# nikizadehgfdl/ocean_model_grid_generator

Measured on AMD Instinct MI355X. Metric: supergrid cells/sec (coords+metrics), 1/8° tripolar at 1/2/4/8 MI355X, higher is better.
Workload: dtype f64

## Files before the change

### ocean_model_grid_generator_amd/csrc/ogg_bipolar_dev.h

```cpp
#pragma once
#include <cstdlib>

#include "ogg_common.h"
#include "ogg_math.h"

namespace {

using namespace ogg;

struct BpRow {
    double sphig;
    double beta2_inv;
    double N_inv;
};
struct BpCol {
    double sinla;
    double alpha2;
};

OGG_DEV BpRow bp_row(double phig_in, double rp) {
    BpRow r;
    const double phig = 90 - div_pi180(2 * atan(tan(0.5 * (90 - phig_in) * kPi180) / rp));
    const double pr = phig * kPi180;
    r.sphig = sin(pr);
    const double t = tan(pr);
    r.beta2_inv = t * t;
    const double chig = (90 - phig) * kPi180;
    const double tg = tan(chig / 2);
    const double rden2 = 1.0 / (1 + (rp * tg) * (rp * tg));
    const double N = rp * (1 + tg * tg) * rden2;
    r.N_inv = 1 / N;
    return r;
}

OGG_DEV BpCol bp_col(double lamg, double lon_bp) {
    BpCol c;
    const double tmp = mdist(lamg, lon_bp) * kPi180;
    double s, co;
    sincos(tmp, &s, &co);
    c.sinla = s;
    c.alpha2 = co * co;
    return c;
}

OGG_DEV void bp_point(const BpRow& r, const BpCol& c, double rp, double& phis, double& h_i_inv, double& h_j_inv, double& rden_out) {
    const double rden = 1.0 / (1.0 + c.alpha2 * r.beta2_inv);
    const double A = c.sinla * r.sphig;
    const double chic = acos(A);
    const double t = tan(chic / 2);
    const double rpt = rp * t;
    phis = 90 - div_pi180(2 * atan(rpt));
    const double rden2 = 1.0 / (1 + rpt * rpt);
    const double M_inv = rp * (1 + t * t) * rden2;
    const double cp = cos(phis * kPi180);
    const double cos2phis = cp * cp;
    const double MM = M_inv * M_inv;
    const bool huge = fabs(r.beta2_inv) > kHuge;
    const double rr = rden * rden;
    double hj = cos2phis * c.alpha2 * (1 - c.alpha2) * r.beta2_inv * (1 + r.beta2_inv) * rr + MM * (1 - c.alpha2) * rden;
    if (huge) hj = MM;
    h_j_inv = sqrt(hj) * r.N_inv;
    double hi = cos2phis * (1 + r.beta2_inv) * rr + MM * c.alpha2 * r.beta2_inv * rden;
    if (huge) hi = MM;
    h_i_inv = sqrt(hi);
    rden_out = rden;
}

template <bool GUARD>
OGG_DEV bool bp_point_fast(const BpRow& r, double b1, double bb1, const BpCol& c, double a1, double aa1, double rp2p, double rp2m,
                           double guard_kk, double& q, double& Xn, double& Yn) {
    const double ab = c.alpha2 * r.beta2_inv;
    const double A = c.sinla * r.sphig;
    const double P = 1.0 + ab;
    const double D = fma(rp2m, A, rp2p);
    const double mp = fma(-A, A, 1.0);
    q = P * D;
    Xn = fma(aa1, fma(mp, bb1, r.beta2_inv), a1);
    Yn = fma(ab, P, mp * b1);
    if (!GUARD) return false;
    const double kc = guard_kk * mp;
    const double uid = (mp * b1) * D, ujd = (mp * (aa1 * bb1)) * D;
    return (uid * uid > kc * (Yn * Yn)) || (ujd * ujd > kc * (Xn * Xn));
}

__constant__ double kAsinPoly[12] = {0x1.5555555555380p-3, 0x1.333333336fd5bp-4, 0x1.6db6db41ce4bdp-5, 0x1.f1c72c668963fp-6,
                                     0x1.6e89f0a0adacfp-6, 0x1.1c6c111dccb70p-6, 0x1.c6fa84b77012bp-7, 0x1.8ed60a300c8d2p-7,
                                     0x1.ab3a098a70509p-8, 0x1.4052137024d6ap-6, -0x1.0a5a378a05eafp-6, 0x1.059859fea6a70p-5};

OGG_DEV double asin_unit(double x) {
    const bool hi = x >= 0.5;
    const double h = fma(x, -0.5, 0.5);
    const double r = hi ? h : x * x;
    const double p = r * horner_scalar<12>(kAsinPoly, r);
    double v = fma(x, p, x);
    if (hi) {
        const double y = __builtin_amdgcn_rsq(h);
        const double g0 = h * y, h0 = y * 0.5;
        const double e = fma(-h0, g0, 0.5);
        const double h1 = fma(h0, e, h0), g1 = fma(g0, e, g0);
        const double d = fma(-g1, g1, h);
        const double s0 = fma(d, h1, g1);
        const bool zero = h == 0.0;
        const double s = zero ? h : s0;
        const double ss = s * s;
        const double sse = fma(s, s, -ss);
        const double t0 = h - ss;
        const double t1 = ((h - t0) - ss) - sse;
        const double num = t0 + t1;
        const double den = s * 2.0;
        const double rc0 = __builtin_amdgcn_rcp(den);
        const double rc1 = fma(fma(-den, rc0, 1.0), rc0, rc0);
        const double rc = fma(fma(-den, rc1, 1.0), rc1, rc1);
        const double q0 = num * rc;
        const double q = fma(fma(-den, q0, num), rc, q0);
        const double c = zero ? 0.0 : q;
        const double sh = s + c;
        const double sl = c - (sh - s);
        const double ph = p * sh;
        const double pl = fma(sl, p, fma(sh, p, -ph));
        const double a = ph + pl;
        const double al = pl - (a - ph);
        const double b = sh + a;
        const double bl = a - (b - sh);
        const double w = (sl + al) + bl;
        const double u = b + w;
        const double ul = w - (u - b);
        constexpr double pio4 = 0x1.921fb54442d18p-1, pio4_lo = 0x1.1a62633145c07p-55;
        const double z = pio4 - u;
        const double zl = (((pio4 - z) - u) + pio4_lo) - ul;
        const double res = z + zl;
        v = (x == 1.0) ? 0x1.921fb54442d18p+0 : res + res;
    }
    return v;
}

OGG_DEV double bp_lamc(const BpRow& r, const BpCol& c, double sqrt_rden) {
    double B = c.sinla * sqrt_rden;
    if (fabs(r.beta2_inv) > kHuge) B = 0.0;
    return div_pi180(asin_unit(B));
}

OGG_DEV double bp_lams_select(double lamc, double lamg, double lon_bp) {
    const double dl = lamg - lon_bp;
    if ((dl > 90) && (dl <= 180)) lamc = 180 - lamc;
    if ((dl > 180) && (dl <= 270)) lamc = 180 + lamc;
    if (dl > 270) lamc = 360 - lamc;
    if (dl == 90) lamc = 90;
    if (dl == 270) lamc = 270;
// ... 329 lines not shown
inline unsigned top_row_blocks(const QuadParams& p) {
    if (p.top_out_row < 0) return 0u;
    const long waves = (p.nx + top_cells<N>() - 1) / top_cells<N>();
    return (unsigned)((waves + 3) / 4);
}

template <int N>
OGG_DEV void bipolar_top_row_body(const QuadParams& p, long w) {
    constexpr int M = N - 1, CW = top_cells<N>();
    const int lane = threadIdx.x & 63;
    const long c0 = w * CW;
    if (c0 >= p.nx) return;
    long u = M * c0 + lane;
    if (u > M * p.nx) u = M * p.nx;
    const double iv = lattice_node(p.q, (int)(u % M), u / M);
    const double lon = p.lon_bp + (iv * 360.0) / (double)p.nx;
    const BpCol c = bp_col(lon, p.lon_bp);
    const double jv = lattice_node(p.q, 0, p.ny);
    const double latg = p.lat0_bp + (jv * (90 - p.lat0_bp)) / (double)p.ny;
    const BpRow r = bp_row(latg, p.rp);
    double phis, rden, h_i, h_j;
    bp_point(r, c, p.rp, phis, h_i, h_j, rden);
    const double dx = h_i * 2 * kPi / (double)p.nx;
    double y[N];
#pragma unroll
    for (int k = 0; k < N; ++k) y[k] = __shfl_down(dx, k);
    const int cell = lane / M;
    if (lane % M == 0 && cell < CW && c0 + cell < p.nx) p.dxq[p.top_out_row * p.nx + c0 + cell] = quad_average_1d<N>(y) * p.Re;
}

template <int N>
OGG_DEV void bipolar_tables_body(const QuadParams& p, long bx) {
    constexpr int M = N - 1;
    const long nb_tab = tables_only_blocks<N>(p);
    if (bx >= nb_tab) {
        bipolar_top_row_body<N>(p, (bx - nb_tab) * 4 + (threadIdx.x >> 6));
        return;
    }
    BpRow* row_tab = const_cast<BpRow*>(p.row_tab);
    BpCol* col_tab = const_cast<BpCol*>(p.col_tab);
    const long k = bx * blockDim.x + threadIdx.x;
    const long n_rows = M * p.ny + 2, n_cols = M * p.nx + 1;
    if (k == 0) *p.fix_count = 0u;
    for (long w = k; w < QUAD_LL_CLAIM_WORDS; w += nb_tab * blockDim.x) p.ll_claims[w] = 0u;
    if (k < n_rows) {
        double jv;
        if (k == M * p.ny)
            jv = (double)p.ny - 0.001;
        else if (k == M * p.ny + 1)
            jv = lattice_node(p.q, 0, p.ny);
        else
            jv = lattice_node(p.q, (int)(k % M), k / M);
        const double latg = p.lat0_bp + (jv * (90 - p.lat0_bp)) / (double)p.ny;
        row_tab[k] = bp_row(latg, p.rp);
    } else if (k < n_rows + n_cols) {
        const long u = k - n_rows;
        const double iv = lattice_node(p.q, (int)(u % M), u / M);
        const double lon = p.lon_bp + (iv * 360.0) / (double)p.nx;
        col_tab[u] = bp_col(lon, p.lon_bp);
    }
}

template <int N>
__global__ __launch_bounds__(256) void bipolar_tables_kernel(QuadParams p) {
    bipolar_tables_body<N>(p, blockIdx.x);
}

template <int N>
inline unsigned tables_blocks(const QuadParams& p) {
    return tables_only_blocks<N>(p) + top_row_blocks<N>(p);
}


OGG_DEV void wg_store_aligned(double* __restrict__ dst, int n, const double* buf, int j0, int sgn, int wave, int lane) {
    const int mis = (int)((reinterpret_cast<unsigned long>(dst) >> 3) & 15ul);
    const int j = 64 * wave + lane - mis;
    if (j >= 0 && j < n) dst[j] = buf[j0 + sgn * j];
    const int j2 = 64 * QS_WAVES + lane - mis;
    if (wave == 0 && j2 < n) dst[j2] = buf[j0 + sgn * j2];
}

struct QuadOutLds {
    double v[2][3][QS_WG_CELLS];
};

template <int N, int MODE>
struct RowEval {
    double dx[N];
    double dy0;
    double pr[N];
    int guarded;
};

constexpr int QM_FAST = 0, QM_GUARD = 1, QM_LITERAL = 2;

template <int N, int MODE>
OGG_DEV void eval_lattice_row(const QuadParams& p, const BpRow& r, const BpCol* col, double rp2p, bool want_dx, RowEval<N, MODE>& o) {
    constexpr int M = N - 1;
    constexpr bool FAITHFUL = (MODE == QM_LITERAL);
    if (FAITHFUL) {
#pragma unroll 1
        for (int ii = 0; ii < M; ++ii) {
            BpCol c = col[0];
#pragma unroll
            for (int k = 1; k < M; ++k) {
                c.sinla = (ii == k) ? col[k].sinla : c.sinla;
                c.alpha2 = (ii == k) ? col[k].alpha2 : c.alpha2;
            }
            double phis, rden, h_i, h_j;
            bp_point(r, c, p.rp, phis, h_i, h_j, rden);
            const double dx = h_i * 2 * kPi / (double)p.nx;
            const double dy = h_j * (90 - p.lat0_bp) * kPi180 / (double)p.ny;
#pragma unroll
            for (int k = 0; k < M; ++k) {
                o.dx[k] = (ii == k) ? dx : o.dx[k];
                o.pr[k] = (ii == k) ? dx * dy : o.pr[k];
            }
            if (ii == 0) o.dy0 = dy;
        }
    } else {
        const double b1 = 1 + r.beta2_inv, bb1 = r.beta2_inv * b1, nsy = r.N_inv * p.sy;
        const double cdx = p.cdx, cdy = (2 * p.rp) * nsy, cpr = p.rp2x4 * (p.sx * nsy);
        const double guard_kk = p.guard_kk, rp2m = p.rp2m;
        int g_first = 0, g_any = 0;
#pragma unroll
        for (int ii = 0; ii < M; ++ii) {
            double q, Xn, Yn;
            const double a1 = 1 - col[ii].alpha2;
            const bool g = bp_point_fast<MODE == QM_GUARD>(r, b1, bb1, col[ii], a1, col[ii].alpha2 * a1, rp2p, rp2m, guard_kk, q, Xn, Yn);
            if (ii == 0) g_first = g;
            g_any |= (int)g;
            const double q2 = q * q;
            constexpr double tiny = 1e-290;
            if (ii == 0 || want_dx) {
                const double dx = (Yn * rsqrt_c3(Yn * q2)) * cdx;
                const double dy = (Xn * rsqrt_c3(fmax(Xn * q2, tiny))) * cdy;
                o.dx[ii] = dx;
                o.pr[ii] = dx * dy;
                if (ii == 0) o.dy0 = dy;
            } else {
                const double xy = Xn * Yn;
                o.pr[ii] = (xy * rsqrt_c3(fmax(xy * (q2 * q2), tiny))) * cpr;
            }
        }
        o.guarded = 0;
        if (MODE == QM_GUARD) o.guarded = g_any | wave_next(g_first);
    }
    if (FAITHFUL) o.guarded = 0;
    if (FAITHFUL || want_dx) o.dx[M] = wave_next(o.dx[0]);
    o.pr[M] = wave_next(o.pr[0]);
}

template <int N, int MODE>
OGG_DEV void bipolar_quad_body(const QuadParams& p, const QuadRange& rg, QuadOutLds& out, long wgx, long by) {
    constexpr int M = N - 1;
    constexpr bool FAITHFUL = (MODE == QM_LITERAL);
    const int lane = threadIdx.x & 63, wave = threadIdx.x >> 6;
    const QuadLane ql = quad_lane(rg.cols, wgx, wave, lane);
    if (ql.nv == 0) return;
    const bool active = ql.active;
    const long ci = ql.ci, c0 = ql.c0;
    const int nv = ql.nv;
    const long n_cols_tab = M * p.nx + 1;
    BpCol col[M];
#pragma unroll
    for (int ii = 0; ii < M; ++ii) {
        long u = M * ci + ii;
        if (u > n_cols_tab - 1) u = n_cols_tab - 1;
        col[ii] = p.col_tab[u];
    }
    const bool cell_lane = ql.cell_lane, closing = ql.closing;
    const bool img_col = (MODE == QM_FAST) && ql.img_col;
    const long h2 = p.nx / 2;
    const QuadStores qs = quad_stores(rg.cols, ql, p.nx, MODE == QM_FAST);
    double rp2p = p.rp2p;
    asm volatile("" : "+v"(rp2p));
    RowEval<N, MODE> cur;
    const long r0 = rg.row_begin + by * rg.rows_per_chunk;
    const long r1 = (r0 + rg.rows_per_chunk < rg.row_end) ? r0 + rg.rows_per_chunk : rg.row_end;
    if (active) eval_lattice_row<N, MODE>(p, p.row_tab[(long)M * r0], col, rp2p, true, cur);
    const int slot = wave * QS_CELLS + lane;
    for (long c = r0; c < r1; ++c) {
        double dxq = 0.0, dyq = 0.0, da = 0.0;
        int guarded = 0;
        if (active) {
            dxq = quad_average_1d<N>(cur.dx) * p.Re;
            guarded = cur.guarded;
            double dyc[N];
            double y2[(N <= 3) ? N * N : 1];
            double ysum = 0.0;
#pragma unroll
            for (int k = 0; k < N; ++k) dyc[k] = 0.0;
#pragma unroll((N <= 3 || MODE != QM_LITERAL) ? N : 1)
            for (int jj = 0; jj < N; ++jj) {
                if (jj > 0) {
                    eval_lattice_row<N, MODE>(p, p.row_tab[(long)M * c + jj], col, rp2p, jj == M, cur);
                    guarded |= cur.guarded;
                }
                const double wj = quad_weight_1d<N>(jj);
#pragma unroll
                for (int ii = 0; ii < N; ++ii) {
                    const double pr = cur.pr[ii];
                    if (N <= 3) {
#pragma unroll
                        for (int k = 0; k < N * N; ++k)
                            if (N <= 3 && k == jj * N + ii) y2[(N <= 3) ? k : 0] = pr;
                    } else {
                        if (FAITHFUL)
                            ysum = ysum + (quad_weight_1d<N>(ii) * wj) * pr;
                        else
                            ysum = fma(quad_weight_1d<N>(ii) * wj, pr, ysum);
                    }
                }
#pragma unroll
                for (int k = 0; k < N; ++k) dyc[k] = (jj == k) ? cur.dy0 : dyc[k];
            }
            dyq = quad_average_1d<N>(dyc) * p.Re;
            if (N == 2) {
                const double d = 1.0 / 2.0;
                da = d * d * (y2[0] + y2[1] + y2[(N <= 3) ? N : 0] + y2[(N <= 3) ? N + 1 : 0]);
            } else if (N == 3) {
                const double d = 1.0 / 6.0;
                auto Y = [&](int a, int b) { return y2[(N == 3) ? a * 3 + b : 0]; };
                da = d * d * (Y(0, 0) + Y(0, 2) + Y(2, 0) + Y(2, 2) + 4.0 * (Y(0, 1) + Y(1, 0) + Y(1, 2) + Y(2, 1) + 4.0 * Y(1, 1)));
            } else {
                const double d = (N == 4) ? (1.0 / 12.0) : (1.0 / 180.0);
                da = d * d * ysum;
            }
            da = da * p.Re * p.Re;
        }
        const long out_r = c - p.j0;
        double* __restrict__ rdx = p.dxq + out_r * p.nx;
        double* __restrict__ rdy = p.dyq + out_r * (p.nx + 1);
        double* __restrict__ rda = p.daq + out_r * p.nx;
        if (closing) {
            rdy[ci] = dyq;
            if (img_col) rdy[h2 - ci] = dyq, rdy[h2 + ci] = dyq, rdy[p.nx - ci] = dyq;
        }
        if (cell_lane && MODE == QM_GUARD && guarded) p.fix_list[atomicAdd(p.fix_count, 1u)] = (unsigned)(out_r * p.nx + ci);
        double(*buf)[QS_WG_CELLS] = out.v[(c - r0) & 1];
        if (lane < QS_CELLS) buf[0][slot] = dxq, buf[1][slot] = dyq, buf[2][slot] = da;
        __syncthreads();
        wg_store_aligned(rdx + c0, nv, buf[0], 0, 1, wave, lane);
        wg_store_aligned(rdy + c0, nv, buf[1], 0, 1, wave, lane);
        wg_store_aligned(rda + c0, nv, buf[2], 0, 1, wave, lane);
        const int last = nv - 1;
        if (qs.n_ic > 0) {
            wg_store_aligned(rdx + qs.cell_up, qs.n_ic, buf[0], qs.k0, 1, wave, lane);
            wg_store_aligned(rda + qs.cell_up, qs.n_ic, buf[2], qs.k0, 1, wave, lane);
            wg_store_aligned(rdx + qs.cell_dn2, qs.n_ic, buf[0], last, -1, wave, lane);
            wg_store_aligned(rda + qs.cell_dn2, qs.n_ic, buf[2], last, -1, wave, lane);
            wg_store_aligned(rdx + qs.cell_dn4, qs.n_ic, buf[0], last, -1, wave, lane);
            wg_store_aligned(rda + qs.cell_dn4, qs.n_ic, buf[2], last, -1, wave, lane);
        }
        if (qs.n_ip > 0) {
            wg_store_aligned(rdy + qs.col_up, qs.n_ip, buf[1], qs.k1, 1, wave, lane);
            wg_store_aligned(rdy + qs.col_dn2, qs.n_ip, buf[1], last, -1, wave, lane);
            wg_store_aligned(rdy + qs.col_dn4, qs.n_ip, buf[1], last, -1, wave, lane);
        }
    }
}

template <int N, int MODE>
__global__ __launch_bounds__(64 * QS_WAVES) void bipolar_quad_kernel(QuadParams p, QuadRange rg) {
    __shared__ QuadOutLds out;
    bipolar_quad_body<N, MODE>(p, rg, out, blockIdx.x, blockIdx.y);
}

template <int N>
__global__ __launch_bounds__(64) void bipolar_quad_tail_kernel(QuadParams p) {
    constexpr int M = N - 1;
    __shared__ double sdx[64], sdy[64];
    const unsigned bid = blockIdx.x, nblk = gridDim.x;
    const unsigned count = *p.fix_count;
    const int lane = threadIdx.x, half = lane >> 5, q = lane & 31;
    if (p.top_src && p.top_out_row >= 0)
        for (long i = (long)bid * 64 + lane; i < p.nx; i += (long)nblk * 64) p.dxq[p.top_out_row * p.nx + i] = p.top_src[i];
    const int jj = (q < N * N) ? q / N : 0, ii = (q < N * N) ? q % N : 0;
    for (unsigned k0 = bid * 2; k0 < count; k0 += nblk * 2) {
        const unsigned k = k0 + half;
        const bool have = k < count;
        const unsigned lin = have ? p.fix_list[k] : 0u;
        const long out_r = lin / p.nx, ci = lin % p.nx;
        const long cj = p.j0 + out_r;
        double dx = 0.0, dy = 0.0;
        if (have && q < N * N) {
            const BpRow r = p.row_tab[M * cj + jj];
            const BpCol c = p.col_tab[M * ci + ii];
            double phis, rden, h_i, h_j;
            bp_point(r, c, p.rp, phis, h_i, h_j, rden);
            dx = h_i * 2 * kPi / (double)p.nx;
            dy = h_j * (90 - p.lat0_bp) * kPi180 / (double)p.ny;
        }
        __syncthreads();
        sdx[lane] = dx;
        sdy[lane] = dy;
        __syncthreads();
        if (!have || q != 0) continue;
        const int base = half << 5;
        double dxrow[N], dycol[N], dyright[N], y2[(N <= 3) ? N * N : 1];
        double ysum = 0.0;
#pragma unroll
        for (int a = 0; a < N; ++a) {
#pragma unroll
            for (int b = 0; b < N; ++b) {
                const double vx = sdx[base + a * N + b], vy = sdy[base + a * N + b];
                if (a == 0) dxrow[b] = vx;
                if (b == 0) dycol[a] = vy;
                if (b == N - 1) dyright[a] = vy;
                if (N <= 3)
                    y2[(N <= 3) ? a * N + b : 0] = vx * vy;
                else
                    ysum = ysum + (quad_weight_1d<N>(b) * quad_weight_1d<N>(a)) * (vx * vy);
            }
        }
        p.dxq[out_r * p.nx + ci] = quad_average_1d<N>(dxrow) * p.Re;
        p.dyq[out_r * (p.nx + 1) + ci] = quad_average_1d<N>(dycol) * p.Re;
        if (ci == p.nx - 1) p.dyq[out_r * (p.nx + 1) + p.nx] = quad_average_1d<N>(dyright) * p.Re;
        double da;
        if (N == 2) {
            const double d = 1.0 / 2.0;
            da = d * d * (y2[0] + y2[1] + y2[(N <= 3) ? N : 0] + y2[(N <= 3) ? N + 1 : 0]);
        } else if (N == 3) {
            const double d = 1.0 / 6.0;
            auto Y = [&](int a, int b) { return y2[(N == 3) ? a * 3 + b : 0]; };
            da = d * d * (Y(0, 0) + Y(0, 2) + Y(2, 0) + Y(2, 2) + 4.0 * (Y(0, 1) + Y(1, 0) + Y(1, 2) + Y(2, 1) + 4.0 * Y(1, 1)));
        } else {
            const double d = (N == 4) ? (1.0 / 12.0) : (1.0 / 180.0);
            da = d * d * ysum;
        }
        p.daq[out_r * p.nx + ci] = da * p.Re * p.Re;
    }
}

__global__ void bipolar_ij_kernel(long n_i, const double* __restrict__ iv, long n_j, const double* __restrict__ jv, long Ni,
                                  long Nj, double lat0_bp, double lon_bp, double rp, double* __restrict__ hi,
                                  double* __restrict__ hj) {
    const long k = (long)blockIdx.x * blockDim.x + threadIdx.x;
    const long r = blockIdx.y;
    if (k >= n_i || r >= n_j) return;
    const double lon = lon_bp + (iv[k] * 360.0) / (double)Ni;
    const double lat = lat0_bp + (jv[r] * (90 - lat0_bp)) / (double)Nj;
    const BpRow row = bp_row(lat, rp);
    const BpCol col = bp_col(lon, lon_bp);
    double phis, h_i, h_j, rden;
    bp_point(row, col, rp, phis, h_i, h_j, rden);
    hi[r * n_i + k] = h_i * 2 * kPi / (double)Ni;
    hj[r * n_i + k] = h_j * (90 - lat0_bp) * kPi180 / (double)Nj;
}

QuadNodes make_nodes(int order) {
    QuadNodes q{};
    if (order == 2) {
        double a[] = {0.0, 1.0}, b[] = {1.0, 0.0};
        for (int k = 0; k < 2; ++k) q.a[k] = a[k], q.b[k] = b[k];
    } else if (order == 3) {
        double a[] = {0.0, 0.5, 1.0}, b[] = {1.0, 0.5, 0.0};
        for (int k = 0; k < 3; ++k) q.a[k] = a[k], q.b[k] = b[k];
    } else if (order == 4) {
        const double r5 = 0.5 / sqrt(5.0);
        double a[] = {0.0, 0.5 - r5, 0.5 + r5, 1.0}, b[] = {1.0, 0.5 + r5, 0.5 - r5, 0.0};
        for (int k = 0; k < 4; ++k) q.a[k] = a[k], q.b[k] = b[k];
    } else if (order == 5) {
        const double r37 = 0.5 * sqrt(3.0 / 7.0);
        double a[] = {0.0, 0.5 - r37, 0.5, 0.5 + r37, 1.0}, b[] = {1.0, 0.5 + r37, 0.5, 0.5 - r37, 0.0};
        for (int k = 0; k < 5; ++k) q.a[k] = a[k], q.b[k] = b[k];
    }
    return q;
}

template <int N>
size_t quad_workspace_bytes(long nx, long ny, long n_cell_rows) {
    constexpr int M = N - 1;
    const size_t tabs = (size_t)(M * ny + 2) * sizeof(BpRow) + (size_t)(M * nx + 1) * sizeof(BpCol);
    const size_t lists = tabs + 16 + QUAD_LL_CLAIM_WORDS * sizeof(unsigned) + (size_t)(n_cell_rows > 0 ? n_cell_rows : 0) * nx * sizeof(unsigned);
    return (lists + 7) / 8 * 8 + (size_t)nx * sizeof(double);
}

struct QuadPlan {
    QuadParams p;
    bool has_fast, has_guard, has_top;
    QuadRange fast, guard;
    double* top_buf;
};

constexpr double BP_SYM_FOLD_DEG = 6.0;

inline QuadCols quad_cols(long nx, int symmetry) {
    QuadCols c{};
    auto wgs = [](long lo, long hi) { return (hi - lo + QS_WG_CELLS - 1) / QS_WG_CELLS; };
    for (int r = 0; r < 3; ++r) c.lo[r] = c.hi[r] = 0;
    c.lo[0] = 0, c.hi[0] = nx;
    c.g_end[0] = c.g_end[1] = c.g_end[2] = wgs(0, nx);
    c.z = nx, c.sym = 0;
    if (!symmetry || nx % 4 != 0) return c;
    double deg = BP_SYM_FOLD_DEG;
    if (const char* e = getenv("OGG_BP_SYM_FOLD_DEG")) deg = atof(e);
    const long q = nx / 4;
    long z = (long)ceil(deg * (double)nx / 360.0);
    if (z < 1) z = 1;
    if (2 * z > q) return c;
    c.sym = 1, c.z = z;
    c.lo[0] = 0, c.hi[0] = q;
    c.lo[1] = 2 * q - z, c.hi[1] = 2 * q + z;
    c.lo[2] = nx - z, c.hi[2] = nx;
    long g = 0;
    for (int r = 0; r < 3; ++r) g += wgs(c.lo[r], c.hi[r]), c.g_end[r] = g;
    return c;
}

template <int N>
int plan_quad(QuadParams p, long n_dx_rows, long n_cell_rows, double guard_k, int symmetry, void* ws, long ws_bytes, QuadPlan& out) {
    constexpr int M = N - 1;
    const long n_rows = M * p.ny + 2, n_cols = M * p.nx + 1;
    const size_t need = quad_workspace_bytes<N>(p.nx, p.ny, n_cell_rows);
    OGG_REQUIRE(ws && (size_t)ws_bytes >= need, OGG_EARG, "bipolar quadrature workspace too small: %ld < %zu bytes", ws_bytes, need);
    BpRow* row_tab = static_cast<BpRow*>(ws);
    BpCol* col_tab = reinterpret_cast<BpCol*>(row_tab + n_rows);
    unsigned* fix_count = reinterpret_cast<unsigned*>(col_tab + n_cols);
    p.row_tab = row_tab;
    p.col_tab = col_tab;
    p.fix_count = fix_count;
    p.ll_claims = fix_count + 4;
    p.fix_list = fix_count + 4 + QUAD_LL_CLAIM_WORDS;
    p.top_src = nullptr;
    out.top_buf = reinterpret_cast<double*>(static_cast<char*>(ws) + need - (size_t)p.nx * sizeof(double));
    p.guard_k = guard_k;
    p.top_out_row = (n_dx_rows > n_cell_rows) ? n_cell_rows : -1;
    const double rp2 = p.rp * p.rp;
    p.sx = (2 * kPi) / (double)p.nx, p.sy = ((90 - p.lat0_bp) * kPi180) / (double)p.ny;
    p.rp2p = 1 + rp2, p.rp2m = 1 - rp2, p.rp2x4 = 4 * rp2;
    p.cdx = (2 * p.rp) * p.sx;
    p.guard_kk = guard_k * p.rp2x4;
    out.p = p;
    long jg = 0;
    if (guard_k > 4.0) {
        const double lat_thr = acos(2.0 / sqrt(guard_k)) / kPi180;
        jg = (long)floor((double)p.ny * (lat_thr - p.lat0_bp) / (90.0 - p.lat0_bp)) - 1;
    }
    if (jg < 0) jg = 0;
    if (jg > p.ny) jg = p.ny;
    const long lo = p.j0, hi = p.j0 + n_cell_rows;
    auto range = [&](long b, long e, int sym) {
        QuadRange r{};
        r.row_begin = b;
        r.row_end = e;
        r.cols = quad_cols(p.nx, sym);
        r.gx = (unsigned)r.cols.g_end[2];
        long n_strips = 0;
        for (int k = 0; k < 3; ++k) n_strips += (r.cols.hi[k] - r.cols.lo[k] + QS_CELLS - 1) / QS_CELLS;
        long target = 4096;
        if (const char* ev = getenv("OGG_QUAD_TARGET_WAVES")) target = atol(ev) > 0 ? atol(ev) : target;
        long rpc = ((e - b) * n_strips + target - 1) / target;
        r.rows_per_chunk = rpc < 1 ? 1 : (rpc > 32 ? 32 : rpc);
        r.gy = (unsigned)((e - b + r.rows_per_chunk - 1) / r.rows_per_chunk);
        return r;
    };
    out.has_fast = lo < hi && lo < jg;
    out.has_guard = lo < hi && hi > jg;
    out.has_top = n_dx_rows > n_cell_rows;
    if (out.has_fast) out.fast = range(lo, hi < jg ? hi : jg, symmetry);
    if (out.has_guard) out.guard = range(lo > jg ? lo : jg, hi, 0);
    return OGG_OK;
}

constexpr unsigned FIXUP_BLOCKS = 2048;

template <int N>
int launch_quad_tail(const QuadPlan& q, hipStream_t s) {
    if (!q.has_guard && !(q.p.top_src && q.has_top)) return OGG_OK;
    bipolar_quad_tail_kernel<N><<<FIXUP_BLOCKS, 64, 0, s>>>(q.p);
    OGG_LAUNCH_CHECK();
    return OGG_OK;
}

template <int N>
int launch_quad(QuadParams p, long n_dx_rows, long n_cell_rows, double guard_k, int symmetry, void* ext_ws, long ext_ws_bytes, hipStream_t s) {
    const size_t need = quad_workspace_bytes<N>(p.nx, p.ny, n_cell_rows);
    void* ws = ext_ws;
    long ws_bytes = ext_ws_bytes;
    ogg::AsyncScratch own(s);
    if (!ext_ws) {
        if (int e = own.alloc(&ws, need)) return e;
        ws_bytes = (long)need;
    }
    QuadPlan q;
    if (int e = plan_quad<N>(p, n_dx_rows, n_cell_rows, guard_k, symmetry, ws, ws_bytes, q)) return e;
    bipolar_tables_kernel<N><<<tables_blocks<N>(q.p), 256, 0, s>>>(q.p);
    OGG_LAUNCH_CHECK();
    if (q.has_fast) {
        bipolar_quad_kernel<N, QM_FAST><<<dim3(q.fast.gx, q.fast.gy), 64 * QS_WAVES, 0, s>>>(q.p, q.fast);
        OGG_LAUNCH_CHECK();
    }
    if (q.has_guard) {
        bipolar_quad_kernel<N, QM_GUARD><<<dim3(q.guard.gx, q.guard.gy), 64 * QS_WAVES, 0, s>>>(q.p, q.guard);
        OGG_LAUNCH_CHECK();
    }
    return launch_quad_tail<N>(q, s);
}

}
```

### ocean_model_grid_generator_amd/csrc/ogg_math.h

```cpp
#pragma once
#include <hip/hip_runtime.h>

#define OGG_DEV __device__ __forceinline__
#define OGG_HD __host__ __device__ __forceinline__

namespace ogg {

constexpr double kPi = 3.141592653589793;
constexpr double kPi180 = kPi / 180.0;
constexpr double k180Pi = 180.0 / kPi;
constexpr double kHuge = 1.0e30;
constexpr double kReDefault = 6371.0e3;

OGG_DEV double pymod360(double a) {
    double r;
    if (fabs(a) < 1.0e12) {
        double q = floor(a * (1.0 / 360.0));
        r = fma(-q, 360.0, a);
        if (r < 0.0) {
            q -= 1.0;
            r = fma(-q, 360.0, a);
        } else if (r >= 360.0) {
            const double r2 = fma(-(q + 1.0), 360.0, a);
            r = (r2 >= 0.0) ? r2 : r;
// ... 179 lines not shown
    OGG_DEV void keep() const {
#pragma unroll
        for (int i = 0; i < 20; ++i) asm volatile("" ::"v"(k[i]));
    }
};

template <class C>
OGG_DEV double atanred_lib(double v, const C& c) {
    const double t = v * v;
    return fma(v, t * c.eval(t), v);
}

template <class C>
OGG_DEV double atan_lib(double x, const C& c) {
    const double v = fabs(x);
    const bool g = v > 1.0;
    const double a = atanred_lib(g ? 1.0 / v : v, c);
    const double r = g ? fma(0x1.dd9ad336a0500p-1, 0x1.af154eeb562d6p+0, -a) : a;
    return copysign(r, x);
}

template <class C>
OGG_DEV double atan_lib_wave(double x, const C& c) {
    if (__builtin_expect(__ballot(fabs(x) > 1.0) != 0ull, 0)) return atan_lib(x, c);
    return copysign(atanred_lib(fabs(x), c), x);
}

template <class C>
OGG_DEV double atan2_lib(double y, double x, const C& c) {
    const double ay = fabs(y), ax = fabs(x);
    const double mx = fmax(ax, ay), mn = fmin(ax, ay);
    double a = atanred_lib(mn / mx, c);
    const bool xneg = __double2hiint(x) < 0;
    a = (ax < ay) ? 0x1.921fb54442d18p+0 - a : a;
    a = xneg ? 0x1.921fb54442d18p+1 - a : a;
    a = (y == 0.0) ? (xneg ? 0x1.921fb54442d18p+1 : 0.0) : a;
    return copysign(a, y);
}

template <class C>
OGG_DEV double atan2_lib_any(double y, double x, const C& c) {
    double a = atan2_lib(y, x, c);
    const bool xinf = fabs(x) == __builtin_inf(), yinf = fabs(y) == __builtin_inf();
    const double q = (__double2hiint(x) < 0) ? 0x1.2d97c7f3321d2p+1 : 0x1.921fb54442d18p-1;
    a = (xinf && yinf) ? copysign(q, y) : a;
    return (x != x || y != y) ? __builtin_nan("") : a;
}

OGG_DEV double atan_lib(double x) {
    AtanCoefs c;
    c.load(kAtanRed);
    const double r = atan_lib(x, c);
    c.keep();
    return r;
}
OGG_DEV double atan2_lib(double y, double x) {
    AtanCoefs c;
    c.load(kAtanRed);
    const double r = atan2_lib(y, x, c);
    c.keep();
    return r;
}
OGG_DEV double atan2_lib_any(double y, double x) {
    AtanCoefs c;
    c.load(kAtanRed);
    const double r = atan2_lib_any(y, x, c);
    c.keep();
    return r;
}

OGG_DEV double wave_prev(double x) {
    int lo = __double2loint(x), hi = __double2hiint(x);
    lo = __builtin_amdgcn_update_dpp(lo, lo, 0x138, 0xf, 0xf, false);
    hi = __builtin_amdgcn_update_dpp(hi, hi, 0x138, 0xf, 0xf, false);
    return __hiloint2double(hi, lo);
}
OGG_DEV double wave_next(double x) {
    int lo = __double2loint(x), hi = __double2hiint(x);
    lo = __builtin_amdgcn_update_dpp(lo, lo, 0x130, 0xf, 0xf, false);
    hi = __builtin_amdgcn_update_dpp(hi, hi, 0x130, 0xf, 0xf, false);
    return __hiloint2double(hi, lo);
}
OGG_DEV int wave_next(int x) { return __builtin_amdgcn_update_dpp(x, x, 0x130, 0xf, 0xf, false); }

OGG_DEV long xcd_contiguous(long b, long n) {
    const long x = b % 8, r = n % 8;
    return x * (n / 8) + ((x < r) ? x : r) + b / 8;
}

struct QuadNodes {
    double a[5];
    double b[5];
};

OGG_DEV double lattice_node(const QuadNodes& q, int k, long c) {
    return q.b[k] * (double)c + q.a[k] * (double)(c + 1);
}

}
```

### ocean_model_grid_generator_amd/csrc/ogg_pass.hip

```cpp
#include <cstring>
#include <new>
#include <vector>

#include "ogg_bipolar_dev.h"
#include "ogg_dpole_dev.h"
#include "ogg_latlon_fused_dev.h"

extern "C" long ogg_dpole_band_workspace_bytes(int order, long Ni, long n_pt_rows);

namespace {

constexpr int PASS_TX = 256;
static_assert(PASS_TX == LF_TX && PASS_TX == 64 * MESH_WAVES && PASS_TX == 64 * QS_WAVES && PASS_TX == 64 * DM_WAVES &&
                  PASS_TX == 64 * DQ_WAVES,
              "one workgroup shape for all roles");

struct LatlonShare {
    long n_wg;
    long gx, gy;
    long strip_lo, strip_hi;
    int nt;
    unsigned* claims;
    long n_help;
    int pool;
// ... 300 lines not shown
        double guard_k = BP_GUARD_K_DEFAULT;
        if (const char* e = getenv("OGG_BP_GUARD_K")) guard_k = atof(e);
        QuadParams p{};
        p.nx = cap->Ni, p.ny = cap->Nj, p.lat0_bp = cap->lat0_bp, p.lon_bp = cap->lon_bp, p.rp = cap->rp, p.Re = cap->Re, p.j0 = cap->j0;
        p.dxq = cap->dx, p.dyq = cap->dy, p.daq = cap->area, p.q = make_nodes(N);
        if (int e = plan_quad<N>(p, cap->n_pt_rows, cap->n_cell_rows, guard_k, ogg::cap_symmetry(cap->symmetry) ? 1 : 0, cap->workspace,
                                 cap->workspace_bytes, qp))
            return e;
        A.q = qp.p, B.q = qp.p;
        A.n_tab = tables_blocks<N>(qp.p);
        B.guard = qp.guard, B.n_guard = qp.has_guard ? (long)qp.guard.gx * qp.guard.gy : 0;
        B.fast = qp.fast, B.n_fast = qp.has_fast ? (long)qp.fast.gx * qp.fast.gy : 0;
    }
    DpQuadParams& dq = P.dq;
    if (have_dp) {
        const DpGeom g{scap->Ni, scap->Nj, scap->lon0, scap->lat0, scap->lon_dp, scap->r_dp};
        const long mesh_ws = (long)((dm_workspace_bytes(scap->Ni, scap->n_pt_rows) + 255) / 256 * 256);
        OGG_REQUIRE(scap->workspace && scap->workspace_bytes >= mesh_ws, OGG_EARG, "ogg_supergrid_pass: displaced-pole workspace too small");
        if (int e = plan_dmesh(g, scap->j0, scap->n_pt_rows, scap->x, scap->y, scap->angle, scap->workspace, mesh_ws, B.dm)) return e;
        A.dm = B.dm;
        A.n_dm_reset = dm_reset_blocks(B.dm);
        B.n_dmesh = dm_blocks(B.dm);
        if (have_dquad) {
            if (int e = plan_dquad(scap->arc_form, scap->order, g, scap->Re, scap->j0, scap->n_pt_rows, scap->n_cell_rows, scap->dx, scap->dy,
                                   scap->area, static_cast<char*>(scap->workspace) + mesh_ws, scap->workspace_bytes - mesh_ws,
                                   make_nodes(scap->order), dq, ogg::cap_symmetry(scap->symmetry) ? 1 : 0))
                return e;
            A.dq = dq, A.dq_order = scap->order;
            A.n_dq_tab = scap->order == 2 ? dpole_quad_tables_blocks<2>(dq) : dpole_quad_tables_blocks<4>(dq);
            if (!dq_literal) B.dq = dq, B.dq_order = scap->order, B.n_dquad = dq.gx * dq.n_chunks;
            P.dq_order = scap->order;
        }
    }
    const bool launch_b = (have_quad && (B.n_guard + B.n_fast > 0)) || have_dp;
    const long s1 = launch_b ? 0 : n_strips_ll;
    if (launch_b) {
        B.mesh = A.mesh, B.mesh_gx = A.mesh_gx, B.n_mesh = A.n_mesh;
        A.n_mesh = 0;
    }
    {
        const double ni = (double)(ni1 - 1);
        const double mesh_bytes = have_cap ? 8.0 * 3.0 * (double)cap->n_pt_rows * (double)ni1 : 0.0;
        const double bq_bytes = have_quad ? 8.0 * (double)cap->n_cell_rows * (3.0 * ni + 1.0) : 0.0;
        P.alg_bytes[0] = latlon_strip_bytes(ll, 0, s1) + (launch_b ? 0.0 : mesh_bytes) + ((have_quad && qp.has_top) ? 8.0 * ni : 0.0);
        P.alg_bytes[1] = launch_b ? latlon_strip_bytes(ll, s1, n_strips_ll) + bq_bytes + mesh_bytes + (have_dp ? dpole_mesh_bytes(*scap) : 0.0) +
                                        ((have_dquad && !dq_literal) ? dpole_quad_bytes(*scap) : 0.0)
                                  : 0.0;
        P.alg_bytes[2] = 0.0;
        P.alg_bytes[3] = dq_literal ? dpole_quad_bytes(*scap) : 0.0;
    }
    A.share = make_share(ll, 0, s1, ni1, !have_cap && !have_dp);
    if (!(launch_b && ll.row_tab && n_strips_ll > 0)) A.ll.row_tab = nullptr, B.ll.row_tab = nullptr;
    A.n_ll_tab = B.ll.row_tab ? latlon_row_table_blocks(ll) : 0;
    P.na = (unsigned)(A.share.n_wg + A.n_tab + A.n_dq_tab + A.n_dm_reset + A.n_ll_tab + A.n_mesh);
    if (launch_b) {
        static const int quad_first[N_ROLES] = {ROLE_BP_FAST, ROLE_BP_GUARD, ROLE_DP_QUAD, ROLE_BP_MESH, ROLE_DP_MESH};
        static const int mesh_first[N_ROLES] = {ROLE_BP_MESH, ROLE_DP_MESH, ROLE_BP_GUARD, ROLE_BP_FAST, ROLE_DP_QUAD};
        const double quad_cells = (have_quad ? (double)cap->n_cell_rows * (double)cap->Ni : 0.0) +
                                  ((have_dquad && !dq_literal) ? (double)scap->n_cell_rows * (double)scap->Ni : 0.0);
        const int* dflt = quad_cells >= 2.0e6 ? quad_first : mesh_first;
        const char* ord = getenv("OGG_PASS_ORDER");
        for (int k = 0; k < N_ROLES; ++k)
            B.order[k] = (ord && strlen(ord) == N_ROLES && ord[k] >= '0' && ord[k] < '0' + N_ROLES) ? ord[k] - '0' : dflt[k];
        const bool light = have_cap && ogg::cap_symmetry(cap->symmetry) && B.n_dquad == 0;
        B.share = make_share(ll, s1, n_strips_ll, ni1, false, light, have_quad ? -1 : 0);
        if (B.share.pool && B.ll.row_tab && !getenv("OGG_LL_ROWS_PER_STRIP")) {
            const long rpb = env_long("OGG_PASS_LL_ROWS_TABLE", 6);
            if (rpb > 0 && rpb != B.ll.rows_per_block) {
                set_rows_per_strip(B.ll, rpb), set_rows_per_strip(A.ll, rpb);
                B.share = make_share(B.ll, 0, B.ll.strip0[B.ll.n_bands], ni1, false, light, have_quad ? -1 : 0, true);
            }
        }
        const long helpers = env_long("OGG_PASS_LL_HELPERS", (B.share.points >= 16000000 && !light) ? 2 : 0);
        if (B.share.pool && B.share.n_wg > 0 && B.share.gx <= QUAD_LL_CLAIM_WORDS) {
            B.share.claims = qp.p.ll_claims;
            B.share.n_help = B.share.n_wg * env_long("OGG_PASS_LL_POOL_HELPERS", (light || B.ll.row_tab) ? 0 : 1);
        } else if (B.share.pool) {
            B.share.pool = 0;
        } else if (have_quad && helpers > 0 && B.share.n_wg > 0 && 2 * B.share.n_wg <= QUAD_LL_CLAIM_WORDS) {
            B.share.claims = qp.p.ll_claims;
            B.share.n_help = B.share.n_wg * helpers;
        }
        P.nb = (unsigned)(B.share.n_wg + B.n_mesh + B.n_dmesh + B.n_guard + B.n_fast + B.n_dquad + B.share.n_help);
        P.b_lds_pad = (unsigned)env_long("OGG_PASS_B_LDS_PAD", (B.ll.row_tab && light && B.share.points >= 16000000) ? 41000 : 0);
    }
    P.nd = dq_literal ? (unsigned)(dq.gx * dq.n_chunks) : 0u;
    P.have_quad = have_quad, P.dq_literal = dq_literal, P.launch_b = launch_b;
    return OGG_OK;
}

template <int N>
int run_pass_plan(const PassPlan& P, hipEvent_t* ev, double* alg_bytes4, hipStream_t st, bool with_a = true, const PassAParams* next = nullptr,
                  long n_next = 0) {
    auto mark = [&](int k) -> int {
        if (ev && ev[k]) OGG_HIP_CHECK(hipEventRecord(ev[k], st));
        return OGG_OK;
    };
    if (alg_bytes4)
        for (int k = 0; k < 4; ++k) alg_bytes4[k] = P.alg_bytes[k];
    if (int e = mark(0)) return e;
    if (P.na > 0 && with_a) {
        pass_a_kernel<N><<<P.na, PASS_TX, 0, st>>>(P.A);
        OGG_LAUNCH_CHECK();
    }
    if (int e = mark(1)) return e;
    if (P.launch_b) {
        PassBParams b = P.B;
        if (next && n_next > 0) b.next = next, b.n_next = n_next;
        if (b.ll.row_tab)
            pass_b_kernel<N, true><<<P.nb + (unsigned)b.n_next, PASS_TX, P.b_lds_pad, st>>>(b);
        else
            pass_b_kernel<N, false><<<P.nb + (unsigned)b.n_next, PASS_TX, 0, st>>>(b);
        OGG_LAUNCH_CHECK();
    }
    if (int e = mark(2)) return e;
    if (P.have_quad) {
        if (int e = launch_quad_tail<N>(P.qp, st)) return e;
    }
    if (int e = mark(3)) return e;
    if (P.dq_literal) {
        if (P.dq_order == 2)
            pass_d_kernel<2><<<P.nd, PASS_TX, 0, st>>>(P.dq);
        else
            pass_d_kernel<4><<<P.nd, PASS_TX, 0, st>>>(P.dq);
        OGG_LAUNCH_CHECK();
    }
    return mark(4);
}

int build_pass_plan_any(int n_latlon, const ogg_latlon_band* latlon, long ni1, double lon0, double lenlon, double Re, int metrics,
                        const ogg_bipolar_band* cap, const ogg_dpole_band* south_cap, PassPlan& P, const RowScalars* row_tab = nullptr) {
    FusedParams ll;
    long points = 0;
    if (int e = plan_latlon(n_latlon, latlon, ni1, lon0, lenlon, Re, metrics, ll, points)) return e;
    ll.row_tab = row_tab;
    int order = 5;
    if (cap && cap->n_pt_rows > 0) {
        OGG_REQUIRE(cap->Ni + 1 == ni1, OGG_ESHAPE, "ogg_tripolar_pass: cap has %ld columns, the lat-lon bands %ld", cap->Ni + 1, ni1);
        OGG_REQUIRE(cap->Nj > 0 && cap->j0 >= 0 && cap->j0 + cap->n_pt_rows <= cap->Nj + 1, OGG_ESHAPE,
                    "ogg_tripolar_pass: cap rows %ld..%ld outside 0..%ld", cap->j0, cap->j0 + cap->n_pt_rows, cap->Nj);
        OGG_REQUIRE(cap->x && cap->y && cap->angle, OGG_EARG, "ogg_tripolar_pass: null cap output");
        if (metrics) {
            order = cap->order;
            OGG_REQUIRE(order >= 2 && order <= 5, OGG_EORDER, "Uncoded order");
            OGG_REQUIRE(cap->dx && (cap->n_cell_rows <= 0 || (cap->dy && cap->area)), OGG_EARG, "ogg_tripolar_pass: null cap metrics output");
            OGG_REQUIRE(cap->n_cell_rows >= 0 && cap->j0 + cap->n_cell_rows <= cap->Nj &&
                            (cap->n_pt_rows == cap->n_cell_rows ||
                             (cap->n_pt_rows == cap->n_cell_rows + 1 && cap->j0 + cap->n_cell_rows == cap->Nj)),
                        OGG_ESHAPE, "ogg_tripolar_pass: cap band j0=%ld cell rows=%ld point rows=%ld of Nj=%ld", cap->j0,
                        cap->n_cell_rows, cap->n_pt_rows, cap->Nj);
            OGG_REQUIRE(cap->workspace, OGG_EARG, "ogg_tripolar_pass: the cap needs a workspace (ogg_bipolar_quad_workspace_bytes)");
        }
    }
    if (south_cap && south_cap->n_pt_rows > 0) {
        const ogg_dpole_band& d = *south_cap;
        OGG_REQUIRE(d.Ni + 1 == ni1, OGG_ESHAPE, "ogg_supergrid_pass: southern cap has %ld columns, the lat-lon bands %ld", d.Ni + 1, ni1);
        OGG_REQUIRE(d.Nj > 0 && d.j0 >= 0 && d.j0 + d.n_pt_rows <= d.Nj + 1, OGG_ESHAPE,
                    "ogg_supergrid_pass: southern cap rows %ld..%ld outside 0..%ld", d.j0, d.j0 + d.n_pt_rows, d.Nj);
        OGG_REQUIRE(d.x && d.y && d.angle, OGG_EARG, "ogg_supergrid_pass: null southern cap output");
        OGG_REQUIRE(d.workspace && d.workspace_bytes >= ogg_dpole_band_workspace_bytes(metrics ? d.order : 4, d.Ni, d.n_pt_rows), OGG_EARG,
                    "ogg_supergrid_pass: the southern cap needs a workspace of ogg_dpole_band_workspace_bytes bytes");
        if (metrics) {
            OGG_REQUIRE(d.order >= 2 && d.order <= 5, OGG_EORDER, "Uncoded order");
            OGG_REQUIRE(d.order == 2 || d.order == 4, OGG_EORDER, "order not coded");
            OGG_REQUIRE(d.arc_form == OGG_DP_ARC_LITERAL || d.arc_form == OGG_DP_ARC_CHORD, OGG_EARG, "ogg_supergrid_pass: arc_form %d", d.arc_form);
            OGG_REQUIRE(d.dx && (d.n_cell_rows <= 0 || (d.dy && d.area)), OGG_EARG, "ogg_supergrid_pass: null southern cap metrics output");
            OGG_REQUIRE(d.n_cell_rows >= 0 && d.j0 + d.n_cell_rows <= d.Nj &&
// ... 287 lines not shown
```

Measured before the change: 123.2 billion.

## Patch guarded quadrature cells inline instead of deferring to a fixup tail kernel

Guarded cells are no longer appended to a global fix list through an atomic counter. Each wave now ballots them into LDS flags, and the workgroup re-evaluates those cells right after the row barrier: it calls the literal bp_point through a noinline helper and gathers the quadrature points with shuffles. The tail kernel shrinks to copying the top row, which removes a separate launch, the atomics and a second global write pass. In exchange every guarded row pays an extra barrier, a reload of the column table and a recomputation of the next lattice row, plus more code in the main kernel. The LDS pad default is lowered slightly to make room for the new flag array.

```diff
diff --git a/ocean_model_grid_generator_amd/csrc/ogg_bipolar_dev.h b/ocean_model_grid_generator_amd/csrc/ogg_bipolar_dev.h
--- a/ocean_model_grid_generator_amd/csrc/ogg_bipolar_dev.h
+++ b/ocean_model_grid_generator_amd/csrc/ogg_bipolar_dev.h
@@ -64,6 +64,18 @@
     if (huge) hi = MM;
     h_i_inv = sqrt(hi);
     rden_out = rden;
+}
+
+struct BpScale {
+    double h_i_inv, h_j_inv;
+};
+__device__ __attribute__((noinline)) BpScale bp_point_call(double sphig, double beta2_inv, double N_inv, double sinla, double alpha2, double rp) {
+    const BpRow r{sphig, beta2_inv, N_inv};
+    const BpCol c{sinla, alpha2};
+    double phis, rden;
+    BpScale s;
+    bp_point(r, c, rp, phis, s.h_i_inv, s.h_j_inv, rden);
+    return s;
 }
 
 template <bool GUARD>
@@ -559,7 +571,100 @@
 
 struct QuadOutLds {
     double v[2][3][QS_WG_CELLS];
-};
+    unsigned long long flag[2][QS_WAVES];
+};
+
+OGG_DEV int nth_set_bit(unsigned long long m, int n) {
+    int pos = 0;
+#pragma unroll
+    for (int w = 32; w >= 1; w >>= 1) {
+        const int c = __popcll(m & (((1ull << w) - 1ull) << pos));
+        if (n >= c) n -= c, pos += w;
+    }
+    return pos;
+}
+
+struct LiteralCell {
+    double dxq, dyq, dyq_right, daq;
+};
+template <int N>
+OGG_DEV LiteralCell literal_cell_gather(double dx, double dy, int base, double Re) {
+    double dxrow[N], dycol[N], dyright[N], y2[(N <= 3) ? N * N : 1];
+    double ysum = 0.0;
+#pragma unroll
+    for (int a = 0; a < N; ++a) {
+#pragma unroll
+        for (int b = 0; b < N; ++b) {
+            const double vx = __shfl(dx, base + a * N + b), vy = __shfl(dy, base + a * N + b);
+            if (a == 0) dxrow[b] = vx;
+            if (b == 0) dycol[a] = vy;
+            if (b == N - 1) dyright[a] = vy;
+            if (N <= 3)
+                y2[(N <= 3) ? a * N + b : 0] = vx * vy;
+            else
+                ysum = ysum + (quad_weight_1d<N>(b) * quad_weight_1d<N>(a)) * (vx * vy);
+        }
+    }
+    LiteralCell o;
+    o.dxq = quad_average_1d<N>(dxrow) * Re;
+    o.dyq = quad_average_1d<N>(dycol) * Re;
+    o.dyq_right = quad_average_1d<N>(dyright) * Re;
+    double da;
+    if (N == 2) {
+        const double d = 1.0 / 2.0;
+        da = d * d * (y2[0] + y2[1] + y2[(N <= 3) ? N : 0] + y2[(N <= 3) ? N + 1 : 0]);
+    } else if (N == 3) {
+        const double d = 1.0 / 6.0;
+        auto Y = [&](int a, int b) { return y2[(N == 3) ? a * 3 + b : 0]; };
+        da = d * d * (Y(0, 0) + Y(0, 2) + Y(2, 0) + Y(2, 2) + 4.0 * (Y(0, 1) + Y(1, 0) + Y(1, 2) + Y(2, 1) + 4.0 * Y(1, 1)));
+    } else {
+        const double d = (N == 4) ? (1.0 / 12.0) : (1.0 / 180.0);
+        da = d * d * ysum;
+    }
+    o.daq = da * Re * Re;
+    return o;
+}
+
+template <int N>
+OGG_DEV bool quad_patch_row(const QuadParams& p, long c, long c0, const unsigned long long* flag, double (*buf)[QS_WG_CELLS], double* rdy) {
+    constexpr int M = N - 1;
+    static_assert(QS_WAVES == 4, "four ballots per row");
+    if ((flag[0] | flag[1] | flag[2] | flag[3]) == 0ull) return false;
+    int tid = threadIdx.x;
+    asm volatile("" : "+v"(tid));
+    const int q = tid & 31, base = tid & 32, group = tid >> 5;
+    for (int k0 = 0;; k0 += 2 * QS_WAVES) {
+        asm volatile("" ::: "memory");
+        const unsigned long long f0 = flag[0], f1 = flag[1], f2 = flag[2], f3 = flag[3];
+        const int n0 = __popcll(f0), n1 = n0 + __popcll(f1), n2 = n1 + __popcll(f2), total = n2 + __popcll(f3);
+        if (k0 >= total) break;
+        const int k = k0 + group;
+        const bool have = k < total;
+        const int w = (k >= n2) ? 3 : ((k >= n1) ? 2 : ((k >= n0) ? 1 : 0));
+        const unsigned long long m = (w == 3) ? f3 : ((w == 2) ? f2 : ((w == 1) ? f1 : f0));
+        const int below = (w == 3) ? n2 : ((w == 2) ? n1 : ((w == 1) ? n0 : 0));
+        const int slot = have ? w * QS_CELLS + nth_set_bit(m, k - below) : 0;
+        const long ci = c0 + slot;
+        double dx = 0.0, dy = 0.0;
+        if (have && q < N * N) {
+            const int jj = q / N, ii = q % N;
+            const BpRow r = p.row_tab[M * c + jj];
+            const BpCol cc = p.col_tab[M * ci + ii];
+            const BpScale s = bp_point_call(r.sphig, r.beta2_inv, r.N_inv, cc.sinla, cc.alpha2, p.rp);
+            long nx = p.nx, ny = p.ny;
+            double lat0 = p.lat0_bp;
+            asm volatile("" : "+s"(nx), "+s"(ny), "+s"(lat0));
+            dx = s.h_i_inv * 2 * kPi / (double)nx;
+            dy = s.h_j_inv * (90 - lat0) * kPi180 / (double)ny;
+        }
+        const LiteralCell v = literal_cell_gather<N>(dx, dy, base, p.Re);
+        if (have && q == 0) {
+            buf[0][slot] = v.dxq, buf[1][slot] = v.dyq, buf[2][slot] = v.daq;
+            if (ci == p.nx - 1) rdy[p.nx] = v.dyq_right;
+        }
+    }
+    return true;
+}
 
 template <int N, int MODE>
 struct RowEval {
@@ -640,12 +745,15 @@
     const int nv = ql.nv;
     const long n_cols_tab = M * p.nx + 1;
     BpCol col[M];
-#pragma unroll
-    for (int ii = 0; ii < M; ++ii) {
-        long u = M * ci + ii;
-        if (u > n_cols_tab - 1) u = n_cols_tab - 1;
-        col[ii] = p.col_tab[u];
-    }
+    auto load_cols = [&](long cell) {
+#pragma unroll
+        for (int ii = 0; ii < M; ++ii) {
+            long u = M * cell + ii;
+            if (u > n_cols_tab - 1) u = n_cols_tab - 1;
+            col[ii] = p.col_tab[u];
+        }
+    };
+    load_cols(ci);
     const bool cell_lane = ql.cell_lane, closing = ql.closing;
     const bool img_col = (MODE == QM_FAST) && ql.img_col;
     const long h2 = p.nx / 2;
@@ -656,7 +764,6 @@
     const long r0 = rg.row_begin + by * rg.rows_per_chunk;
     const long r1 = (r0 + rg.rows_per_chunk < rg.row_end) ? r0 + rg.rows_per_chunk : rg.row_end;
     if (active) eval_lattice_row<N, MODE>(p, p.row_tab[(long)M * r0], col, rp2p, true, cur);
-    const int slot = wave * QS_CELLS + lane;
     for (long c = r0; c < r1; ++c) {
         double dxq = 0.0, dyq = 0.0, da = 0.0;
         int guarded = 0;
@@ -710,14 +817,38 @@
         double* __restrict__ rdx = p.dxq + out_r * p.nx;
         double* __restrict__ rdy = p.dyq + out_r * (p.nx + 1);
         double* __restrict__ rda = p.daq + out_r * p.nx;
-        if (closing) {
+        const int par = (int)((c - r0) & 1);
+        bool closed_by_patch = false;
+        if (MODE == QM_GUARD) {
+            const int flagged = (cell_lane && guarded) ? 1 : 0;
+            const unsigned long long wave_flags = __ballot(flagged);
+            if (lane == 0) out.flag[par][wave] = wave_flags;
+            closed_by_patch = wave_prev(flagged) != 0;
+        }
+        if (closing && !closed_by_patch) {
             rdy[ci] = dyq;
             if (img_col) rdy[h2 - ci] = dyq, rdy[h2 + ci] = dyq, rdy[p.nx - ci] = dyq;
         }
-        if (cell_lane && MODE == QM_GUARD && guarded) p.fix_list[atomicAdd(p.fix_count, 1u)] = (unsigned)(out_r * p.nx + ci);
-        double(*buf)[QS_WG_CELLS] = out.v[(c - r0) & 1];
-        if (lane < QS_CELLS) buf[0][slot] = dxq, buf[1][slot] = dyq, buf[2][slot] = da;
+        double(*buf)[QS_WG_CELLS] = out.v[par];
+        if (lane < QS_CELLS) {
+            int t = threadIdx.x;
+            if (MODE == QM_GUARD) asm volatile("" : "+v"(t));
+            const int slot = (t >> 6) * QS_CELLS + (t & 63);
+            buf[0][slot] = dxq, buf[1][slot] = dyq, buf[2][slot] = da;
+        }
         __syncthreads();
+        if (MODE == QM_GUARD) {
+            if (quad_patch_row<N>(p, c, c0, out.flag[par], buf, rdy)) {
+                __syncthreads();
+                int t = threadIdx.x;
+                asm volatile("" : "+v"(t));
+                load_cols(c0 + (long)(t >> 6) * QS_CELLS + (t & 63));
+                if (active)
+                    eval_lattice_row<N, MODE>(p, p.row_tab[(long)M * (c + 1)], col, rp2p, true, cur);
+                else
+                    cur = RowEval<N, MODE>{};
+            }
+        }
         wg_store_aligned(rdx + c0, nv, buf[0], 0, 1, wave, lane);
         wg_store_aligned(rdy + c0, nv, buf[1], 0, 1, wave, lane);
         wg_store_aligned(rda + c0, nv, buf[2], 0, 1, wave, lane);
@@ -745,69 +876,10 @@
 }
 
 template <int N>
-__global__ __launch_bounds__(64) void bipolar_quad_tail_kernel(QuadParams p) {
-    constexpr int M = N - 1;
-    __shared__ double sdx[64], sdy[64];
-    const unsigned bid = blockIdx.x, nblk = gridDim.x;
-    const unsigned count = *p.fix_count;
-    const int lane = threadIdx.x, half = lane >> 5, q = lane & 31;
-    if (p.top_src && p.top_out_row >= 0)
-        for (long i = (long)bid * 64 + lane; i < p.nx; i += (long)nblk * 64) p.dxq[p.top_out_row * p.nx + i] = p.top_src[i];
-    const int jj = (q < N * N) ? q / N : 0, ii = (q < N * N) ? q % N : 0;
-    for (unsigned k0 = bid * 2; k0 < count; k0 += nblk * 2) {
-        const unsigned k = k0 + half;
-        const bool have = k < count;
-        const unsigned lin = have ? p.fix_list[k] : 0u;
-        const long out_r = lin / p.nx, ci = lin % p.nx;
-        const long cj = p.j0 + out_r;
-        double dx = 0.0, dy = 0.0;
-        if (have && q < N * N) {
-            const BpRow r = p.row_tab[M * cj + jj];
-            const BpCol c = p.col_tab[M * ci + ii];
-            double phis, rden, h_i, h_j;
-            bp_point(r, c, p.rp, phis, h_i, h_j, rden);
-            dx = h_i * 2 * kPi / (double)p.nx;
-            dy = h_j * (90 - p.lat0_bp) * kPi180 / (double)p.ny;
-        }
-        __syncthreads();
-        sdx[lane] = dx;
-        sdy[lane] = dy;
-        __syncthreads();
-        if (!have || q != 0) continue;
-        const int base = half << 5;
-        double dxrow[N], dycol[N], dyright[N], y2[(N <= 3) ? N * N : 1];
-        double ysum = 0.0;
-#pragma unroll
-        for (int a = 0; a < N; ++a) {
-#pragma unroll
-            for (int b = 0; b < N; ++b) {
-                const double vx = sdx[base + a * N + b], vy = sdy[base + a * N + b];
-                if (a == 0) dxrow[b] = vx;
-                if (b == 0) dycol[a] = vy;
-                if (b == N - 1) dyright[a] = vy;
-                if (N <= 3)
-                    y2[(N <= 3) ? a * N + b : 0] = vx * vy;
-                else
-                    ysum = ysum + (quad_weight_1d<N>(b) * quad_weight_1d<N>(a)) * (vx * vy);
-            }
-        }
-        p.dxq[out_r * p.nx + ci] = quad_average_1d<N>(dxrow) * p.Re;
-        p.dyq[out_r * (p.nx + 1) + ci] = quad_average_1d<N>(dycol) * p.Re;
-        if (ci == p.nx - 1) p.dyq[out_r * (p.nx + 1) + p.nx] = quad_average_1d<N>(dyright) * p.Re;
-        double da;
-        if (N == 2) {
-            const double d = 1.0 / 2.0;
-            da = d * d * (y2[0] + y2[1] + y2[(N <= 3) ? N : 0] + y2[(N <= 3) ? N + 1 : 0]);
-        } else if (N == 3) {
-            const double d = 1.0 / 6.0;
-            auto Y = [&](int a, int b) { return y2[(N == 3) ? a * 3 + b : 0]; };
-            da = d * d * (Y(0, 0) + Y(0, 2) + Y(2, 0) + Y(2, 2) + 4.0 * (Y(0, 1) + Y(1, 0) + Y(1, 2) + Y(2, 1) + 4.0 * Y(1, 1)));
-        } else {
-            const double d = (N == 4) ? (1.0 / 12.0) : (1.0 / 180.0);
-            da = d * d * ysum;
-        }
-        p.daq[out_r * p.nx + ci] = da * p.Re * p.Re;
-    }
+__global__ __launch_bounds__(256) void bipolar_quad_tail_kernel(QuadParams p) {
+    if (!(p.top_src && p.top_out_row >= 0)) return;
+    for (long i = (long)blockIdx.x * blockDim.x + threadIdx.x; i < p.nx; i += (long)gridDim.x * blockDim.x)
+        p.dxq[p.top_out_row * p.nx + i] = p.top_src[i];
 }
 
 __global__ void bipolar_ij_kernel(long n_i, const double* __restrict__ iv, long n_j, const double* __restrict__ jv, long Ni,
@@ -941,12 +1013,11 @@
     return OGG_OK;
 }
 
-constexpr unsigned FIXUP_BLOCKS = 2048;
-
 template <int N>
 int launch_quad_tail(const QuadPlan& q, hipStream_t s) {
     if (!q.has_guard && !(q.p.top_src && q.has_top)) return OGG_OK;
-    bipolar_quad_tail_kernel<N><<<FIXUP_BLOCKS, 64, 0, s>>>(q.p);
+    const unsigned blocks = (q.p.top_src && q.has_top) ? (unsigned)((q.p.nx + 255) / 256) : 1u;
+    bipolar_quad_tail_kernel<N><<<blocks, 256, 0, s>>>(q.p);
     OGG_LAUNCH_CHECK();
     return OGG_OK;
 }
diff --git a/ocean_model_grid_generator_amd/csrc/ogg_math.h b/ocean_model_grid_generator_amd/csrc/ogg_math.h
--- a/ocean_model_grid_generator_amd/csrc/ogg_math.h
+++ b/ocean_model_grid_generator_amd/csrc/ogg_math.h
@@ -285,6 +285,7 @@
     return __hiloint2double(hi, lo);
 }
 OGG_DEV int wave_next(int x) { return __builtin_amdgcn_update_dpp(x, x, 0x130, 0xf, 0xf, false); }
+OGG_DEV int wave_prev(int x) { return __builtin_amdgcn_update_dpp(x, x, 0x138, 0xf, 0xf, false); }
 
 OGG_DEV long xcd_contiguous(long b, long n) {
     const long x = b % 8, r = n % 8;
diff --git a/ocean_model_grid_generator_amd/csrc/ogg_pass.hip b/ocean_model_grid_generator_amd/csrc/ogg_pass.hip
--- a/ocean_model_grid_generator_amd/csrc/ogg_pass.hip
+++ b/ocean_model_grid_generator_amd/csrc/ogg_pass.hip
@@ -406,7 +406,7 @@
             B.share.n_help = B.share.n_wg * helpers;
         }
         P.nb = (unsigned)(B.share.n_wg + B.n_mesh + B.n_dmesh + B.n_guard + B.n_fast + B.n_dquad + B.share.n_help);
-        P.b_lds_pad = (unsigned)env_long("OGG_PASS_B_LDS_PAD", (B.ll.row_tab && light && B.share.points >= 16000000) ? 41000 : 0);
+        P.b_lds_pad = (unsigned)env_long("OGG_PASS_B_LDS_PAD", (B.ll.row_tab && light && B.share.points >= 16000000) ? 40936 : 0);
     }
     P.nd = dq_literal ? (unsigned)(dq.gx * dq.n_chunks) : 0u;
     P.have_quad = have_quad, P.dq_literal = dq_literal, P.launch_b = launch_b;
```

After: 129.3 billion (median of 6 runs). 1.05x the previous value.
